# Indra-jith/failure-aware-vision

Hardware: AMD Instinct MI355X
Metric: frames/sec, ResNet-50 MC-Dropout T=30 224x224 batch=256 (higher is better)
Workload: dtype bf16; 1 GPU; BASELINE configs[2]: ResNet-50 v1.5 + MC-Dropout T=30 (all_blocks, p=0.10), 224x224x3 fp32 frames with Gaussian noise severity 3, batch 256 per GPU, synthetic frames and seeded synthetic weights; frames_per_gpu=256, global_batch=256, mc_samples=30, dropout_policy=all_blocks, inputs=resident in HBM before the timed region (H2D excluded), parallelism=batch sharded, 1 process per GPU, all-gather of (label, confidence)

## Files before the change

failure_aware_vision_amd/_lib.py:

```python
from __future__ import annotations

import ctypes as C
import os

_HERE = os.path.dirname(os.path.abspath(__file__))
LIB_PATH = os.environ.get("FAV_LIB_PATH") or os.path.join(_HERE, "lib", "libfav_hip.so")

FAV_OK = 0
STATUS_NAMES = {0: "FAV_OK", 1: "FAV_ERR_INVALID_ARG", 2: "FAV_ERR_BAD_BLOB", 3: "FAV_ERR_NO_WEIGHTS",
                4: "FAV_ERR_HIP", 5: "FAV_ERR_NO_DEVICE", 6: "FAV_ERR_UNSUPPORTED"}
LAYOUT_NHWC_U8, LAYOUT_NHWC_F32 = 0, 1
ARCH_RESNET18_CIFAR, ARCH_RESNET50, ARCH_VIT_B16, ARCH_VIT_TINY = 0, 1, 2, 3
CONF_MAX_SOFTMAX, CONF_ENTROPY, CONF_MUTUAL_INFO = 0, 1, 2
MATH_BF16, MATH_F32_EXACT = 0, 1
K_STEM, K_CONV, K_MAXPOOL, K_AVGPOOL, K_DROPOUT, K_HEAD, K_COUNT = 0, 1, 2, 3, 4, 5, 6
KERNEL_CLASS_NAMES = ("stem_im2col", "conv_igemm", "maxpool", "avgpool", "entry_dropout", "head")


class FavConfig(C.Structure):
    _fields_ = [
        ("struct_size", C.c_uint32), ("device", C.c_int32), ("arch", C.c_int32), ("num_classes", C.c_int32),
        ("in_h", C.c_int32), ("in_w", C.c_int32), ("max_batch", C.c_int32),
        ("mean", C.c_float * 3), ("stdev", C.c_float * 3),
        ("n_samples", C.c_int32), ("site_mask", C.c_uint32), ("dropout_p", C.c_float), ("seed", C.c_uint64),
# ... 13 lines not shown
                ("n_frames", C.c_int32), ("H", C.c_int32), ("W", C.c_int32), ("Cin", C.c_int32), ("Cout", C.c_int32),
                ("kh", C.c_int32), ("kw", C.c_int32), ("stride", C.c_int32), ("pad", C.c_int32),
                ("relu", C.c_int32), ("out_f32", C.c_int32), ("math_mode", C.c_int32), ("drop", FavDropoutDesc)]


class FavLinearDesc(C.Structure):
    _fields_ = [("x", C.c_void_p), ("w", C.c_void_p), ("bias", C.c_void_p), ("res", C.c_void_p), ("y", C.c_void_p),
                ("rows", C.c_int64), ("K", C.c_int32), ("N", C.c_int32), ("act", C.c_int32)]


class FavTailDesc(C.Structure):
    _fields_ = [("x", C.c_void_p), ("wb", C.c_void_p), ("bias_b", C.c_void_p), ("wc", C.c_void_p), ("bias_c", C.c_void_p),
                ("res", C.c_void_p), ("y", C.c_void_p), ("wa", C.c_void_p), ("bias_a", C.c_void_p), ("t1n", C.c_void_p),
                ("n_frames", C.c_int32), ("H", C.c_int32), ("W", C.c_int32), ("Cmid", C.c_int32), ("Nred", C.c_int32),
                ("drop", FavDropoutDesc), ("res_entry", C.c_int32), ("entry_site", C.c_int32)]


class FavUncertainty(C.Structure):
    _fields_ = [("label", C.c_int32), ("confidence", C.c_float), ("mean_prob", C.c_float), ("prob_std", C.c_float),
                ("pred_entropy", C.c_float), ("expected_entropy", C.c_float), ("mutual_info", C.c_float),
                ("agreement", C.c_float), ("top_label", C.c_int32 * 5), ("top_prob", C.c_float * 5)]


CP_LAC, CP_APS = 0, 1


class FavConformal(C.Structure):
    _fields_ = [("struct_size", C.c_uint32), ("score_kind", C.c_int32), ("randomized", C.c_int32), ("k_reg", C.c_int32),
                ("lambda_", C.c_float), ("qhat", C.c_float), ("seed", C.c_uint64)]

# ... 32 lines not shown
                                      C.c_void_p, C.c_void_p]),
    "fav_classify_uncertainty": (C.c_int, [C.c_void_p, C.c_void_p, C.c_int32, C.c_int32, C.c_int64, C.c_void_p, C.c_void_p,
                                          C.c_void_p, C.c_void_p]),
    "fav_classify_sets": (C.c_int, [C.c_void_p, C.c_void_p, C.c_int32, C.c_int32, C.c_int64, C.POINTER(FavConformal),
                                    C.c_void_p, C.c_void_p, C.c_void_p, C.c_void_p]),
    "fav_conformal_scores": (C.c_int, [C.c_void_p, C.c_void_p, C.c_int32, C.c_int32, C.c_int64, C.POINTER(FavConformal),
                                       C.c_void_p, C.c_void_p, C.c_void_p]),
    "fav_classify_host": (C.c_int, [C.c_void_p, C.c_void_p, C.c_int32, C.c_int32, C.c_int64, C.c_void_p, C.c_void_p,
                                    C.c_void_p, C.c_void_p]),
    "fav_get_logits": (C.c_int, [C.c_void_p, C.c_void_p, C.POINTER(C.c_int32), C.POINTER(C.c_int32), C.c_void_p]),
    "fav_set_profiling": (C.c_int, [C.c_void_p, C.c_int32]),
    "fav_get_profile": (C.c_int, [C.c_void_p, C.POINTER(FavProfile), C.c_int32]),
    "fav_get_op_profile": (C.c_int, [C.c_void_p, C.POINTER(FavOpProfile), C.c_int32, C.POINTER(C.c_int32)]),
    "fav_op_conv2d": (C.c_int, [C.POINTER(FavConvDesc), C.c_void_p]),
    "fav_op_bottleneck_tail": (C.c_int, [C.POINTER(FavTailDesc), C.c_void_p]),
    "fav_op_linear_streamk": (C.c_int, [C.POINTER(FavLinearDesc), C.c_void_p]),
    "fav_op_stem_im2col": (C.c_int, [C.c_void_p, C.c_int32, C.c_int32, C.c_int32, C.c_int32, C.c_int32, C.c_int32,
                                     C.c_int32, C.c_int32, C.c_int32, C.POINTER(C.c_float), C.POINTER(C.c_float),
                                     C.c_void_p, C.c_void_p]),
    "fav_op_stem_pool": (C.c_int, [C.c_void_p, C.c_int32, C.c_int32, C.c_int32, C.c_int32, C.c_void_p, C.c_void_p, C.c_void_p, C.c_void_p, C.c_void_p, C.c_void_p]),
    "fav_op_maxpool3x3s2": (C.c_int, [C.c_void_p, C.c_void_p, C.c_int32, C.c_int32, C.c_int32, C.c_int32, C.c_void_p]),
    "fav_op_avgpool": (C.c_int, [C.c_void_p, C.c_void_p, C.c_int32, C.c_int32, C.c_int32, C.POINTER(FavDropoutDesc),
                                 C.c_void_p]),
    "fav_op_entry_dropout": (C.c_int, [C.c_void_p, C.c_void_p, C.c_int64, C.c_int32, C.POINTER(FavDropoutDesc),
                                       C.c_void_p]),
    "fav_op_entry_reduce": (C.c_int, [C.c_void_p, C.c_void_p, C.c_void_p, C.c_void_p, C.c_void_p, C.c_int32, C.c_int32, C.c_int32,
                                      C.c_int32, C.POINTER(FavDropoutDesc), C.c_void_p]),
    "fav_op_layernorm": (C.c_int, [C.c_void_p, C.c_int64, C.c_void_p, C.c_void_p, C.c_void_p, C.c_int64, C.c_int32, C.c_float,
                                   C.c_void_p]),
    "fav_op_attention": (C.c_int, [C.c_void_p, C.c_void_p, C.c_int32, C.c_int32, C.c_int32, C.c_int32, C.c_int32, C.c_void_p]),
# ... 42 lines not shown
```

failure_aware_vision_amd/csrc/fav.hip:

```cpp
#include <hip/hip_runtime.h>

#include <algorithm>
#include <atomic>
#include <cmath>
#include <cstdarg>
#include <cstdio>
#include <cstdlib>
#include <cstring>
#include <string>
#include <vector>

#include "../../include/fav.h"
#include "fav_kernels.hpp"

namespace {

thread_local std::string g_create_error;

std::string fmt(const char* f, ...) {
    char buf[512];
    va_list ap;
    va_start(ap, f);
    vsnprintf(buf, sizeof buf, f, ap);
    va_end(ap);
// ... 393 lines not shown
        } else if (epi && pp && MODE_ == 0) hipLaunchKernelGGL((conv_igemm_kernel<256, 256, 64, 2, 0, 2, 0, 1, 1>), grid, dim3(512), 0, s, p); \
        else if (epi) hipLaunchKernelGGL((conv_igemm_kernel<256, 256, 64, 2, MODE_, 2, 0, 1>), grid, dim3(512), 0, s, p);    \
        else hipLaunchKernelGGL((conv_igemm_kernel<256, 256, 64, 2, MODE_, 2, 0, 0>), grid, dim3(512), 0, s, p);        \
    } while (0)
    if (big) {
        if (d.math_mode == FAV_MATH_BF16) FAV_LAUNCH_BIG(0); else FAV_LAUNCH_BIG(1);
    } else if (d.math_mode == FAV_MATH_BF16) FAV_LAUNCH_MODE(0); else FAV_LAUNCH_MODE(1);
#undef FAV_LAUNCH_BIG
#undef FAV_LAUNCH_MODE
#undef FAV_LAUNCH
    dbg_report(tiles, BM, BN, BK);
    return nullptr;
}


struct TailGeom { int patch_bytes, rega_bytes, lds_bytes, nw, wc2, rp, bias_b_off, bias_ca_off, wa_off0, wa_off1, zero_off; };
bool tail_l4() {
    return FAV_KNOB("FAV_TAIL_L4", 1) != 0;
}
bool tail_geometry(int cmid, int nred, bool has3x3, int W, TailGeom* g) {
    const int cout = 4 * cmid;
    auto finish = [&](int bias_b_off, int wa_off0, int wa_bytes) {
        g->bias_b_off = bias_b_off; g->bias_ca_off = bias_b_off + cmid * 5;
        g->wa_off0 = wa_off0; g->wa_off1 = wa_off0 + wa_bytes;
        g->zero_off = (bias_b_off + (cmid + cout + nred) * 5 + 255) & ~255;
        g->lds_bytes = g->zero_off + 256;
    };
    if (cmid == 512) {
        if (has3x3 || nred != 0) return false;
        g->patch_bytes = 0; g->rega_bytes = 0; g->nw = 8; g->rp = 32; g->wc2 = 1;
        finish(2 * 65536, 2 * 65536, 0);
        return true;
    }
    else if (cmid == 256) { if ((has3x3 && nred != 0) || !(nred == 0 || nred == 256)) return false; }
    else if ((cmid != 64 && cmid != 128) || !(nred == 0 || nred == cmid || nred == 128)) return false;
    if (cmid == 256 && has3x3) {
        g->patch_bytes = 0; g->rega_bytes = 128 * 1024; g->nw = 8; g->rp = 32; g->wc2 = 1;
        finish(g->rega_bytes, g->rega_bytes, 0);
        return true;
    }
    const int rp = (cmid == 256 && nred == 256) ? 16 : 32;
    const int rowb = cmid * 2, ns = cmid == 64 ? 3 : 2;
    const int wc_bytes = 64 * rowb, wa_bytes = nred * 128;
    auto plan = [&](int nw) {
        const int bm = rp * nw;
        const int patch = has3x3 ? (int)((((long long)(bm + 2 * W + 2) * rowb) + 1023) / 1024 * 1024) : 0;
        int rega = has3x3 ? std::max(std::max(patch, bm * 128), bm * rowb) : (nred > 0 ? bm * 128 : 0);
        rega = (rega + 1023) / 1024 * 1024;
        const int ring = has3x3 ? ns * cmid * 128 : 0;
        const int budget = nw == 4 ? 80 * 1024 : 160 * 1024;
        g->patch_bytes = patch; g->rega_bytes = rega; g->nw = nw; g->rp = rp;
        g->wc2 = 1;
        int regb = std::max(ring, 2 * wc_bytes + 2 * wa_bytes);
        finish(rega + regb, rega + 2 * wc_bytes, wa_bytes);
        if (g->lds_bytes > budget) {
            g->wc2 = 0;
            regb = std::max(ring, wc_bytes + 2 * wa_bytes);
            finish(rega + regb, rega + wc_bytes, wa_bytes);
        }
        return g->lds_bytes <= budget;
    };
    return plan((cmid == 128 || (cmid == 256 && nred == 256)) ? 8 : 4);
}

bool tail_wide() {
    return FAV_KNOB("FAV_TAIL_WIDE", 1) != 0;
}

bool tail_wide3x3() {
    return FAV_KNOB("FAV_TAIL_WIDE3X3", 1) != 0;
}

bool tail_enabled() {
    return FAV_KNOB("FAV_FUSE", 1) != 0;
}

const char* launch_tail(fav_handle* h, const fav_tail_desc& d, hipStream_t s) {
    const bool has3x3 = d.wb != nullptr;
    const int nred = d.wa ? d.Nred : 0;
    TailGeom g;
    if (!tail_geometry(d.Cmid, nred, has3x3, d.W, &g)) return "bottleneck tail: unsupported shape";
    const long long M = (long long)d.n_frames * d.H * d.W;
    if (M <= 0 || M > 0x7fffffffLL) return "bottleneck tail: row count out of range";
    TailParams p;
    p.t1 = (const uint16_t*)d.x; p.wb = (const uint16_t*)d.wb; p.bias_b = d.bias_b;
    p.wc = (const uint16_t*)d.wc; p.bias_c = d.bias_c; p.res = (const uint16_t*)d.res; p.y = (uint16_t*)d.y;
    p.wa = (const uint16_t*)d.wa; p.bias_a = d.bias_a; p.t1n = (uint16_t*)d.t1n;
    p.H = d.H; p.W = d.W; p.HW = d.H * d.W; p.M = (int)M;
    p.in_W = d.W; p.in_HW = p.HW; p.in_stride = 1;
    p.rega_bytes = g.rega_bytes;
    p.bias_b_off = g.bias_b_off; p.bias_ca_off = g.bias_ca_off; p.wa_off0 = g.wa_off0; p.wa_off1 = g.wa_off1; p.zero_off = g.zero_off;
    p.drop = make_drop(&d.drop);
    p.div_hw = fastdiv_make((uint32_t)p.HW);
    p.div_w = fastdiv_make((uint32_t)d.W);
    if (p.drop.site >= 0 && (p.drop.v0 < 0 || p.drop.v0 + d.n_frames > 0x7fffffffLL)) return "bottleneck tail: virtual frame index out of range";
    const fav_handle::Group G = h ? h->grp : fav_handle::Group{};
// ... 60 lines not shown
        dbg_report();                                                                                                 \
        return nullptr;                                                                                               \
    } while (0)
#define FAV_TAIL_W(CMID_, NRED_, H3_, NS_, NW_) do { if (g.wc2) FAV_TAIL(CMID_, NRED_, H3_, NS_, NW_, true); else FAV_TAIL(CMID_, NRED_, H3_, NS_, NW_, false); } while (0)
#define FAV_TAIL_N(CMID_, NRED_, H3_, NS_) FAV_TAIL_W(CMID_, NRED_, H3_, NS_, 4)
    if (d.res_entry) {
        const bool sample_minor = FAV_KNOB("FAV_ENTRY_RES_ORDER", 1) != 0;
        const long long sample_rows = (long long)p.drop.n_img * p.HW;
        if (sample_minor && p.drop.v0 % p.drop.n_img == 0 && d.n_frames % p.drop.n_img == 0 && sample_rows % bm == 0) {
            p.rs_T = d.n_frames / p.drop.n_img;
            p.rs_tps = (int)(sample_rows / bm);
        }
        static DeviceFlags attr_set;
        auto k0 = bottleneck_tail_kernel<64, 64, true, 3, 4, false, 32, 0, true, true, true>;
        auto k1 = bottleneck_tail_kernel<64, 64, true, 3, 4, true, 32, 0, true, true, true>;
        if (!attr_set.test_current()) {
            if (hipFuncSetAttribute((const void*)k0, hipFuncAttributeMaxDynamicSharedMemorySize, 160 * 1024) != hipSuccess ||
                hipFuncSetAttribute((const void*)k1, hipFuncAttributeMaxDynamicSharedMemorySize, 160 * 1024) != hipSuccess)
                return "bottleneck tail: cannot reserve LDS";
            attr_set.set_current();
        }
        if (g.wc2) hipLaunchKernelGGL(k1, grid, dim3(256), g.lds_bytes, s, p, g.patch_bytes);
        else hipLaunchKernelGGL(k0, grid, dim3(256), g.lds_bytes, s, p, g.patch_bytes);
        dbg_report();
        return nullptr;
    }
    if (cmid == 64) {
        if (has3x3) { if (nred == 0) FAV_TAIL_N(64, 0, true, 3); if (nred == 64) FAV_TAIL_N(64, 64, true, 3); if (nred == 128) FAV_TAIL_N(64, 128, true, 3); }
        else { if (nred == 0) FAV_TAIL_N(64, 0, false, 3); if (nred == 64) FAV_TAIL_N(64, 64, false, 3); if (nred == 128) FAV_TAIL_N(64, 128, false, 3); }
    } else if (cmid == 128) {
        if (has3x3) { if (nred == 0) FAV_TAIL_W(128, 0, true, 2, 8); if (nred == 128) FAV_TAIL_W(128, 128, true, 2, 8); }
        else { if (nred == 0) FAV_TAIL_W(128, 0, false, 2, 8); if (nred == 128) FAV_TAIL_W(128, 128, false, 2, 8); }
    } else if (cmid == 512) {
        FAV_TAIL(512, 0, false, 2, 8, true);
    } else if (nred == 0 && has3x3) {
        FAV_TAIL(256, 0, true, 2, 8, true);
    } else if (nred == 0) {
        FAV_TAIL_W(256, 0, false, 2, 4);
// ... 1494 lines not shown
    return FAV_OK;
}

fav_status fav_op_conv2d(const fav_conv_desc* d, void* stream) {
    if (!d || !d->x || !d->w || !d->bias || !d->y) return op_done("fav_op_conv2d: null pointer");
    if (d->Cout % 64 != 0) return op_done("fav_op_conv2d: Cout must be a multiple of 64");
    return op_done(launch_conv(nullptr, *d, d->Cout, d->Cout, (hipStream_t)stream));
}

fav_status fav_op_bottleneck_tail(const fav_tail_desc* d, void* stream) {
    if (!d || !d->x || !d->wc || !d->bias_c || !d->res || !d->y) return op_done("fav_op_bottleneck_tail: null pointer");
    if ((d->wb && !d->bias_b) || (d->wa && (!d->bias_a || !d->t1n))) return op_done("fav_op_bottleneck_tail: null pointer");
    return op_done(launch_tail(nullptr, *d, (hipStream_t)stream));
}

fav_status fav_op_stem_im2col(const void* images, int32_t layout, int32_t n, int32_t H, int32_t W, int32_t kh, int32_t kw,
                              int32_t stride, int32_t pad, int32_t kpad, const float* mean3, const float* inv_std3,
                              void* out, void* stream) {
    if (!images || !out || !mean3 || !inv_std3 || kpad % 64 != 0 || kpad < kh * kw * 3) return op_done("fav_op_stem_im2col: bad argument");
    launch_stem(nullptr, images, layout, n, H, W, kh, kw, stride, pad, kpad, mean3, inv_std3, out, (hipStream_t)stream);
    return op_done(nullptr);
}

fav_status fav_op_stem_pool(const void* images, int32_t layout, int32_t n, int32_t H, int32_t W, const void* w, const float* bias,
                            const float* mean3, const float* inv_std3, void* out, void* stream) {
    if (!images || !w || !bias || !mean3 || !inv_std3 || !out) return op_done("fav_op_stem_pool: null argument");
    return op_done(launch_stem_pool(nullptr, images, layout, n, H, W, w, bias, mean3, inv_std3, out, (hipStream_t)stream));
}

fav_status fav_op_maxpool3x3s2(const void* x, void* y, int32_t n, int32_t H, int32_t W, int32_t C, void* stream) {
// ... 101 lines not shown
```

failure_aware_vision_amd/csrc/fav_kernels.hpp:

```cpp
#pragma once
#include <hip/hip_runtime.h>
#include <stdint.h>

#ifdef FAV_EXPERIMENTS
#define FAV_DBG(P) ((P).dbg)
#else
#define FAV_DBG(P) ((unsigned long long*)nullptr)
#endif

namespace fav {

typedef __attribute__((__vector_size__(8 * sizeof(__bf16)))) __bf16 bf16x8_t;
typedef __attribute__((__vector_size__(4 * sizeof(float)))) float f32x4_t;

__device__ __forceinline__ float bf16_bits_to_f32(uint32_t b) { return __uint_as_float(b << 16); }

__device__ __forceinline__ uint32_t f32_to_bf16_bits(float f) {
    uint32_t u = __float_as_uint(f);
    return (u + 0x7FFFu + ((u >> 16) & 1u)) >> 16;
}
typedef __bf16 bf16x2_t __attribute__((ext_vector_type(2)));
typedef float f32x2_t __attribute__((ext_vector_type(2)));
typedef uint32_t u32x4_t __attribute__((ext_vector_type(4)));
__device__ __forceinline__ uint32_t pack_bf16x2(float lo, float hi) {
// ... 1215 lines not shown
        asm volatile("s_waitcnt lgkmcnt(0)" ::: "memory");      \
        __builtin_amdgcn_s_barrier();                           \
        asm volatile("" ::: "memory");                          \
    } while (0)

__device__ __forceinline__ int tail_row_perm(int r) {
    const int g = r & ~63, a = (r >> 4) & 3, i = r & 15;
    return g + 16 * (i >> 2) + 4 * a + (i & 3);
}

template <int CPR>
__device__ __forceinline__ int tail_sw(int row) {
    return CPR == 8 ? (row & 7) : (CPR == 16 ? ((row & 7) | ((row & 1) << 3)) : (row & 15));
}

template <int CMID, int NRED, bool HAS3X3, int NS, int NW, bool WC2, int RP = 32, int COUT_ = 0, bool HAS_RES = true, bool RELU = true, bool RESE = false>
__global__ __launch_bounds__(NW * 64, 2) void bottleneck_tail_kernel(const TailParams p_launch, int patch_bytes) {
    const TailParams p = tail_group_params(p_launch);
    constexpr bool LINEST = NRED > 0 || (HAS3X3 && !(HAS3X3 && CMID == 256));
    constexpr int COUT = COUT_ > 0 ? COUT_ : 4 * CMID;
    static_assert(HAS_RES || (!HAS3X3 && NRED == 0), "only conv_c alone runs without a residual");
    constexpr int BM = RP * NW, NT = NW * 64;
    static_assert(RP == 32 || (RP == 16 && !HAS3X3), "rows per wave");
    constexpr int ROWB = CMID * 2;
    constexpr int CPR = ROWB / 16;
    constexpr int PROWS = 1024 / ROWB;
    constexpr int CB = CMID / 64;
    constexpr int NKT = 9 * CB;
    constexpr int TM = 4;
    constexpr int WN1 = 2;
    constexpr int TN1 = CMID / WN1 / 16;
    constexpr int SLOT = CMID * 128;
    constexpr int BR = SLOT / 1024 / NW;
    constexpr int NCHUNK = COUT / 64;
    constexpr int KS2 = CMID / 32;
    constexpr int TM2 = RP / 16;
    constexpr int G3 = NRED / 64;
    constexpr int WC_BYTES = 64 * ROWB;
    constexpr int WA_BYTES = NRED * 128;
    constexpr int WCN = (HAS3X3 && CMID == 256) ? 4 : (WC2 ? 2 : 1);
    constexpr int BARQ = WCN == 4 ? 2 : 1;
    constexpr int P2W = WCN * WC_BYTES + 2 * WA_BYTES;
    constexpr int RING = HAS3X3 ? NS * SLOT : 0;
    constexpr int REGB = RING > P2W ? RING : P2W;
    constexpr int WC_PIECES = WC_BYTES / 1024, WA_PIECES = WA_BYTES / 1024;
    constexpr int WC_PW = (WC_PIECES + NW - 1) / NW, WA_PW = (WA_PIECES + NW - 1) / NW;
    static_assert(BR >= 1 && TN1 >= 1 && TM2 >= 1 && WC_PIECES % NW == 0 && (NRED == 0 || WA_PIECES % NW == 0), "tile shape");
    static_assert(!HAS3X3 || (NKT % NS == 0 && WC_BYTES <= SLOT), "Wc buffer 0 = ring slot 0, free during the last NS - 1 steps");
    const bool WA0_EARLY = !HAS3X3 || p.wa_off1 >= p.rega_bytes + RING;
    constexpr bool P1G = HAS3X3 && CMID == 256;
    static_assert(!P1G || (NW == 8 && NS == 2 && RP == 32 && NRED == 0 && WC2), "generic conv_b: 8 waves, two stages, conv_c alone behind it");
    extern __shared__ __attribute__((aligned(16))) unsigned char tsm[];
    unsigned char* const ych = tsm;
    unsigned char* const regb = P1G ? tsm : tsm + p.rega_bytes;
    float* const bias_b_s = (float*)(tsm + p.bias_b_off);
    float* const bias_c_s = (float*)(tsm + p.bias_ca_off);
    float* const bias_a_s = bias_c_s + (COUT / 16) * 20;
    const uint32_t zero_off = (uint32_t)p.zero_off;

    const int tid = threadIdx.x, lane = tid & 63, wave = tid >> 6;
    const int wm = wave / WN1, wn = wave % WN1;
    const int wave_u = __builtin_amdgcn_readfirstlane(wave);
    const int frow = lane & 15, fq = lane >> 4;
// ... 39 lines not shown
        }                                                                                                         \
    } while (0)
    if (tid < 64) ((uint32_t*)(tsm + zero_off))[tid] = 0u;
    const __amdgpu_buffer_rsrc_t srd_res = RESE
        ? __builtin_amdgcn_make_buffer_rsrc((void*)p.res, 0, (int)((long long)p.drop.n_img * p.HW * COUT * 2), 0x00020000)
        : __builtin_amdgcn_make_buffer_rsrc((void*)((HAS_RES ? p.res : p.y) + (long long)m0 * COUT), 0, rows_valid * COUT * 2, 0x00020000);
    uint32_t eoff[TM2];
    if constexpr (RESE) {
#pragma unroll
        for (int b = 0; b < TM2; ++b) {
            const uint32_t m = (uint32_t)(m0 + wave * RP + b * 16 + frow);
            const uint32_t vl = fastdiv(m, p.div_hw);
            const uint32_t v = (uint32_t)p.drop.v0 + vl;
            const uint32_t il = v - fastdiv(v, p.drop.div_img) * (uint32_t)p.drop.n_img;
            eoff[b] = m < (uint32_t)p.M ? (il * (uint32_t)p.HW + (m - vl * (uint32_t)p.HW)) * (uint32_t)(COUT * 2) : 0x80000000u;
        }
    }
    u32x4_t rnext[TM2][2];
#define FAV_T_LOAD_RES(J)                                                                                        \
    if (HAS_RES) _Pragma("unroll") for (int b = 0; b < TM2; ++b) {                                               \
        const int off = RESE ? (int)(eoff[b] + (uint32_t)(((J) * 64 + fq * 16) * 2))                             \
                             : ((wave * RP + b * 16 + frow) * COUT + (J) * 64 + fq * 16) * 2;                    \
        rnext[b][0] = __builtin_amdgcn_raw_buffer_load_b128(srd_res, off, 0, 0);                                 \
        rnext[b][1] = __builtin_amdgcn_raw_buffer_load_b128(srd_res, off + 16, 0, 0);                            \
    }
    FAV_T_LOAD_RES(0)
    const uint32_t lds_base =
        __builtin_amdgcn_readfirstlane((uint32_t)(uintptr_t)(const __attribute__((address_space(3))) void*)tsm);
    const uint32_t lds_regb = lds_base + (P1G ? 0u : (uint32_t)p.rega_bytes);
    constexpr uint32_t OOB = 0x80000000u;
    const int wrow = lane >> 3, wch = (lane & 7) ^ (wrow & 7);
    const __amdgpu_buffer_rsrc_t srd_wc = __builtin_amdgcn_make_buffer_rsrc((void*)p.wc, 0, COUT * CMID * 2, 0x00020000);
    const __amdgpu_buffer_rsrc_t srd_wa = __builtin_amdgcn_make_buffer_rsrc((void*)p.wa, 0, NRED > 0 ? NRED * COUT * 2 : 16, 0x00020000);
#define FAV_T_STAGE_WC(J)                                                                                        \
    do {                                                                                                         \
        _Pragma("unroll") for (int i = 0; i < WC_PW; ++i) {                                                      \
            const int pc = wave_u + i * NW;                 \
            const int sub = pc >> 3, r0 = (pc & 7) * 8;                                                          \
            lds_dma16(srd_wc, (uint32_t)((((J) * 64 + tail_row_perm(r0 + wrow)) * CMID + sub * 64 + wch * 8) * 2), 0u, \
                      __builtin_amdgcn_readfirstlane(lds_regb + (uint32_t)(((J) % WCN) * WC_BYTES + pc * 1024)));  \
        }                                                                                                        \
    } while (0)
#define FAV_T_STAGE_WA(J)                                                                                        \
    do {                                                                                                         \
        _Pragma("unroll") for (int i = 0; i < WA_PW; ++i) {                                                      \
            const int pc = wave_u + i * NW;                                                                      \
            lds_dma16(srd_wa, (uint32_t)((tail_row_perm(pc * 8 + wrow) * COUT + wch * 8) * 2), (uint32_t)((J) * 128), \
                      __builtin_amdgcn_readfirstlane(lds_base + (uint32_t)(((((J) + 1) & 1) ? p.wa_off1 : p.wa_off0) + pc * 1024))); \
        }                                                                                                        \
    } while (0)

    const int W = p.W;
    if (NRED > 0 && WA0_EARLY) FAV_T_STAGE_WA(0);
    if (HAS3X3) {
        f32x4_t acc[TN1][TM];
// ... 161 lines not shown
#pragma unroll
                    for (int b = 0; b < TM; ++b) {
                        union { uint4 u; bf16x8_t v; } ua, ub;
                        ua.u = fw[a];
                        ub.u = fx[b];
                        acc[a][b] = __builtin_amdgcn_mfma_f32_16x16x32_bf16(ua.v, ub.v, acc[a][b], 0, 0, 0);
                    }
            }
            if (++cb == CB) {
                cb = 0;
                ++tap;
                if (++ts == 3) { ts = 0; ++tr; }
                tapoff = tr * W + ts;
            }
            if (kt + NS - 1 < NKT) asm volatile("s_waitcnt vmcnt(%0)" ::"n"((NS - 2) * BR) : "memory");
            else if (kt + 1 < NKT) asm volatile("s_waitcnt vmcnt(%0)" ::"n"(WC_PW + (NS - 3) * BR) : "memory");
            __syncthreads();
            cur = (cur + 1 == NS) ? 0 : cur + 1;
            nxt = (nxt + 1 == NS) ? 0 : nxt + 1;
        }
#undef FAV_T_HSTAGE
        }
        if (NRED > 0 && !WA0_EARLY) FAV_T_STAGE_WA(0);
        if (FAV_DBG(p) && tid == 0) FAV_DBG(p)[blockIdx.x * 16ull + 2] = wall_clock64();
#pragma unroll
        for (int a = 0; a < TN1; ++a)
#pragma unroll
            for (int b = 0; b < TM; ++b) {
                const int row = wm * 64 + b * 16 + frow;
                const int c0 = wn * (CMID / WN1) + a * 16 + fq * 4;
                const float4 bq = *(const float4*)(bias_b_s + (c0 >> 4) * 20 + (c0 & 15));
// ... 55 lines not shown
    for (int b = 0; b < TM2; ++b) {
        const uint32_t m = (uint32_t)(m0 + wave * RP + b * 16 + frow);
        const uint32_t vl = fastdiv(m, p.div_hw);
        drop_v[b] = (uint32_t)p.drop.v0 + vl;
        drop_pix[b] = m - vl * (uint32_t)p.HW;
    }
    constexpr int NA3 = NRED > 0 ? NRED / 16 : 1;
    f32x4_t acc3[NA3][TM2];
#pragma unroll
    for (int a = 0; a < NA3; ++a)
#pragma unroll
        for (int b = 0; b < TM2; ++b) acc3[a][b] = (f32x4_t){0.f, 0.f, 0.f, 0.f};

#pragma unroll
    for (int j = 0; j < NCHUNK; ++j) {
        const unsigned char* const wcb = regb + (j % WCN) * WC_BYTES;
        const unsigned char* const wab = tsm + (((j + 1) & 1) ? p.wa_off1 : p.wa_off0);
        if ((j == 1 || j == 2) && FAV_DBG(p) && tid == 0) FAV_DBG(p)[blockIdx.x * 16ull + (j == 1 ? 12 : 14)] = __builtin_amdgcn_s_memtime();
        if (HAS_RES) {
#pragma unroll
            for (int b = 0; b < TM2; ++b) {
                asm volatile("" : "+v"(rnext[b][0]), "+v"(rnext[b][1]));
                rcur[b][0] = rnext[b][0];
                rcur[b][1] = rnext[b][1];
            }
        }
        if (j == 1 && FAV_DBG(p) && tid == 0) { asm volatile("s_nop 0" :: "v"(rcur[TM2 - 1][1])); FAV_DBG(p)[blockIdx.x * 16ull + 13] = __builtin_amdgcn_s_memtime(); }
        if (j + 1 < NCHUNK) {
            if (BARQ == 2) {
                if ((j & 1) == 0 && j + 2 < NCHUNK) { FAV_T_STAGE_WC(j + 2); FAV_T_STAGE_WC(j + 3); }
            } else if (WC2) FAV_T_STAGE_WC(j + 1);
            if (NRED > 0) FAV_T_STAGE_WA(j + 1);
            FAV_T_LOAD_RES(j + 1)
        }
        if (j == 1 && FAV_DBG(p) && tid == 0) FAV_DBG(p)[blockIdx.x * 16ull + 6] = __builtin_amdgcn_s_memtime();
        f32x4_t acc2[4][TM2];
#pragma unroll
        for (int a = 0; a < 4; ++a)
#pragma unroll
            for (int b = 0; b < TM2; ++b) acc2[a][b] = (f32x4_t){0.f, 0.f, 0.f, 0.f};
#pragma unroll
        for (int ks = 0; ks < KS2; ++ks) {
            uint4 fw[4];
#pragma unroll
            for (int a = 0; a < 4; ++a) {
                const int row = a * 16 + frow;
                fw[a] = *(const uint4*)(wcb + (ks >> 1) * 8192 + row * 128 + ((((ks & 1) * 4 + fq) ^ (row & 7)) << 4));
            }
#pragma unroll
            for (int a = 0; a < 4; ++a)
#pragma unroll
                for (int b = 0; b < TM2; ++b) {
                    union { uint4 u; bf16x8_t v; } ua, ub;
                    ua.u = fw[a];
                    ub.u = t2f[b][ks];
                    acc2[a][b] = __builtin_amdgcn_mfma_f32_16x16x32_bf16(ua.v, ub.v, acc2[a][b], 0, 0, 0);
                }
        }
        if (j == 1 && FAV_DBG(p) && tid == 0) { asm volatile("s_nop 0" :: "v"(acc2[3][TM2 - 1])); FAV_DBG(p)[blockIdx.x * 16ull + 7] = __builtin_amdgcn_s_memtime(); }
        if (!WC2 && j + 1 < NCHUNK) {
            FAV_BAR();
            FAV_T_STAGE_WC(j + 1);
        }
        {
            float bia[16];
#pragma unroll
            for (int q = 0; q < 4; ++q) {
                const float4 bq = *(const float4*)(bias_c_s + (j * 4 + fq) * 20 + 4 * q);
                bia[4 * q] = bq.x; bia[4 * q + 1] = bq.y; bia[4 * q + 2] = bq.z; bia[4 * q + 3] = bq.w;
            }
#pragma unroll
            for (int b = 0; b < TM2; ++b) {
                const int row = wave * RP + b * 16 + frow;
                const int n = j * 64 + fq * 16;
                uint32_t draws[4] = {~0u, ~0u, ~0u, ~0u};
                uint32_t edraws[4] = {~0u, ~0u, ~0u, ~0u};
                if (p.drop.site >= 0) {
                    const uint32_t chunk = (uint32_t)(((long long)drop_pix[b] * COUT + n) >> 4);
                    const uint4 w4 = drop_draws16(p.drop, drop_v[b], chunk);
                    draws[0] = w4.x; draws[1] = w4.y; draws[2] = w4.z; draws[3] = w4.w;
                    if constexpr (RESE) {
                        DropParams de = p.drop;
                        de.site = p.site_e;
                        const uint4 e4 = drop_draws16(de, drop_v[b], chunk);
                        edraws[0] = e4.x; edraws[1] = e4.y; edraws[2] = e4.z; edraws[3] = e4.w;
                    }
                }
#pragma unroll
                for (int g = 0; g < 2; ++g) {
                    float v[8];
#pragma unroll
                    for (int k = 0; k < 8; ++k) v[k] = __fadd_rn(acc2[2 * g + (k >> 2)][b][k & 3], bia[8 * g + k]);
                    if (HAS_RES) {
                        uint32_t rw[4] = {rcur[b][g][0], rcur[b][g][1], rcur[b][g][2], rcur[b][g][3]};
                        if constexpr (RESE) {
#pragma unroll
                            for (int k = 0; k < 4; ++k) {
                                const float lo = FAV_DROP_APPLY(bf16_bits_to_f32(rw[k] & 0xFFFFu), edraws, 8 * g + 2 * k, p.drop);
                                const float hi = FAV_DROP_APPLY(bf16_bits_to_f32(rw[k] >> 16), edraws, 8 * g + 2 * k + 1, p.drop);
                                rw[k] = pack_bf16x2(lo, hi);
                            }
                        }
#pragma unroll
                        for (int k = 0; k < 4; ++k) {
                            v[2 * k] = __fadd_rn(v[2 * k], bf16_bits_to_f32(rw[k] & 0xFFFFu));
                            v[2 * k + 1] = __fadd_rn(v[2 * k + 1], bf16_bits_to_f32(rw[k] >> 16));
                        }
                    }
                    if (p.drop.site >= 0) {
#pragma unroll
                        for (int k = 0; k < 8; ++k) v[k] = FAV_DROP_APPLY(v[k], draws, 8 * g + k, p.drop);
                    }
                    u32x4_t o = {pack_bf16x2(v[0], v[1]), pack_bf16x2(v[2], v[3]), pack_bf16x2(v[4], v[5]), pack_bf16x2(v[6], v[7])};
                    if (RELU) {
#pragma unroll
                        for (int k = 0; k < 4; ++k) o[k] = relu_bf16x2(o[k]);
                    }
                    if (!LINEST) __builtin_amdgcn_raw_buffer_store_b128(o, srd_y, (row * COUT + n + 8 * g) * 2, 0, 0);
                    if (LINEST) *(u32x4_t*)(ych + row * 128 + (((2 * fq + g) ^ (row & 7)) << 4)) = o;
                }
            }
        }
        if (j == 1 && FAV_DBG(p) && tid == 0) FAV_DBG(p)[blockIdx.x * 16ull + 8] = __builtin_amdgcn_s_memtime();
        if constexpr (LINEST) {
            asm volatile("s_waitcnt lgkmcnt(0)" ::: "memory");
            {
#pragma unroll
                for (int i = 0; i < TM2 * 2; ++i) {
                    const int row = wave * RP + i * 8 + (lane >> 3);
                    const u32x4_t o = *(const u32x4_t*)(ych + row * 128 + (((lane & 7) ^ (row & 7)) << 4));
                    __builtin_amdgcn_raw_buffer_store_b128(o, srd_y, (row * COUT + j * 64 + (lane & 7) * 8) * 2, 0, 0);
                }
            }
        }
        if constexpr (NRED > 0) {
// ... 9 lines not shown
                for (int a = 0; a < NA3; ++a) {
                    const int row = a * 16 + frow;
                    union { uint4 u; bf16x8_t v; } ua;
                    ua.u = *(const uint4*)(wab + row * 128 + (((ks * 4 + fq) ^ (row & 7)) << 4));
#pragma unroll
                    for (int b = 0; b < TM2; ++b) {
                        union { uint4 u; bf16x8_t v; } ub;
                        ub.u = fy[b];
                        acc3[a][b] = __builtin_amdgcn_mfma_f32_16x16x32_bf16(ua.v, ub.v, acc3[a][b], 0, 0, 0);
                    }
                }
            }
        }
        if (j == 1 && FAV_DBG(p) && tid == 0) { asm volatile("s_nop 0" :: "v"(acc3[NA3 - 1][TM2 - 1])); FAV_DBG(p)[blockIdx.x * 16ull + 9] = __builtin_amdgcn_s_memtime(); }
        if (j + 1 < NCHUNK && (BARQ == 1 || (j & 1))) {
            asm volatile("s_waitcnt vmcnt(%0)" ::"n"((WC2 && HAS_RES) ? 4 * TM2 : 2 * TM2) : "memory");
            if (j == 1 && FAV_DBG(p) && tid == 0) FAV_DBG(p)[blockIdx.x * 16ull + 10] = __builtin_amdgcn_s_memtime();
            FAV_BAR();
            if (j == 1 && FAV_DBG(p) && tid == 0) FAV_DBG(p)[blockIdx.x * 16ull + 11] = __builtin_amdgcn_s_memtime();
        }
    }
#undef FAV_T_LOAD_RES
#undef FAV_T_STAGE_WC
#undef FAV_T_STAGE_WA
#undef FAV_T_BIAS_TO_LDS

    if (FAV_DBG(p) && tid == 0) FAV_DBG(p)[blockIdx.x * 16ull + 4] = wall_clock64();
    if constexpr (NRED > 0) {
        const __amdgpu_buffer_rsrc_t srd_t =
            __builtin_amdgcn_make_buffer_rsrc((void*)(p.t1n + (long long)m0 * NRED), 0, rows_valid * NRED * 2, 0x00020000);
#pragma unroll
        for (int g3 = 0; g3 < G3; ++g3) {
            float bia[16];
#pragma unroll
            for (int q = 0; q < 4; ++q) {
                const float4 bq = *(const float4*)(bias_a_s + (g3 * 4 + fq) * 20 + 4 * q);
                bia[4 * q] = bq.x; bia[4 * q + 1] = bq.y; bia[4 * q + 2] = bq.z; bia[4 * q + 3] = bq.w;
// ... 1494 lines not shown
```

include/fav.h:

```cpp
#ifndef FAV_H
#define FAV_H

#include <stddef.h>
#include <stdint.h>

#ifdef __cplusplus
extern "C" {
#endif

#define FAV_ABI_VERSION 2

typedef struct fav_handle fav_handle;

typedef enum fav_status {
    FAV_OK = 0,
    FAV_ERR_INVALID_ARG = 1,
    FAV_ERR_BAD_BLOB = 2,
    FAV_ERR_NO_WEIGHTS = 3,
    FAV_ERR_HIP = 4,
    FAV_ERR_NO_DEVICE = 5,
    FAV_ERR_UNSUPPORTED = 6
} fav_status;

typedef enum fav_layout { FAV_LAYOUT_NHWC_U8 = 0, FAV_LAYOUT_NHWC_F32 = 1 } fav_layout;
// ... 129 lines not shown
fav_status fav_op_conv2d(const fav_conv_desc* d, void* hip_stream);

typedef struct fav_tail_desc {
    const void* x;
    const void* wb; const float* bias_b;
    const void* wc; const float* bias_c;
    const void* res;
    void* y;
    const void* wa; const float* bias_a;
    void* t1n;
    int32_t n_frames, H, W, Cmid, Nred;
    fav_dropout_desc drop;
    int32_t res_entry, entry_site;
} fav_tail_desc;
fav_status fav_op_bottleneck_tail(const fav_tail_desc* d, void* hip_stream);
fav_status fav_op_stem_im2col(const void* images, int32_t layout, int32_t n, int32_t H, int32_t W,
                              int32_t kh, int32_t kw, int32_t stride, int32_t pad, int32_t kpad,
                              const float* mean3, const float* inv_std3, void* out, void* hip_stream);
fav_status fav_op_stem_pool(const void* images, int32_t layout, int32_t n, int32_t H, int32_t W, const void* w, const float* bias,
                            const float* mean3, const float* inv_std3, void* out, void* hip_stream);
fav_status fav_op_maxpool3x3s2(const void* x, void* y, int32_t n, int32_t H, int32_t W, int32_t C, void* hip_stream);
fav_status fav_op_avgpool(const void* x, void* y, int32_t n, int32_t HW, int32_t C,
                          const fav_dropout_desc* drop, void* hip_stream);
fav_status fav_op_entry_dropout(const void* x, void* out, int64_t elems_per_frame, int32_t n_out,
                                const fav_dropout_desc* drop, void* hip_stream);
fav_status fav_op_entry_reduce(const void* x, void* y, const void* wa, const float* bias_a, void* t1, int32_t C, int32_t Nred,
                               int32_t HW, int32_t n_out, const fav_dropout_desc* drop, void* hip_stream);
fav_status fav_op_head(const float* logits, int32_t T, int32_t n, int32_t num_classes, int32_t ld,
                       float temperature, int32_t conf_kind, float tau,
                       int32_t* labels, float* conf, uint8_t* fail, float* score, void* hip_stream);
// ... 44 lines not shown
```

Baseline: 3427 frames/s.

## Add three-blocks-per-CU LDS plan for cmid=64 bottleneck tail kernel

Adds a tighter LDS geometry for the cmid=64, nred=64 bottleneck tail with a 3x3 conv. It uses two ring slots, a single Wc buffer placed in a ring slot, and launch bounds of occupancy 3, so three blocks fit per CU within 160KB of LDS. To keep register pressure down, residual loads move later, per row block, after the conv_c MMA, and Wa staging is deferred with schedule barriers. This is the default path for layer1 shapes, and a knob and API let callers force 2 or 3 blocks. The trade-off is less load latency hiding from the shallower pipeline and a possible register-limit spill under the 3-block bound.

```diff
diff --git a/failure_aware_vision_amd/_lib.py b/failure_aware_vision_amd/_lib.py
--- a/failure_aware_vision_amd/_lib.py
+++ b/failure_aware_vision_amd/_lib.py
@@ -51,6 +51,11 @@
                 ("res", C.c_void_p), ("y", C.c_void_p), ("wa", C.c_void_p), ("bias_a", C.c_void_p), ("t1n", C.c_void_p),
                 ("n_frames", C.c_int32), ("H", C.c_int32), ("W", C.c_int32), ("Cmid", C.c_int32), ("Nred", C.c_int32),
                 ("drop", FavDropoutDesc), ("res_entry", C.c_int32), ("entry_site", C.c_int32)]
+
+
+class FavTailPlan(C.Structure):
+    _fields_ = [(k, C.c_int32) for k in ("lds_bytes", "patch_bytes", "rega_bytes", "waves", "rows_per_wave", "ring_slots", "wc_buffers",
+                                         "blocks_per_cu", "bias_b_off", "bias_ca_off", "wa_off0", "wa_off1", "zero_off")]
 
 
 class FavUncertainty(C.Structure):
@@ -113,6 +118,8 @@
     "fav_get_op_profile": (C.c_int, [C.c_void_p, C.POINTER(FavOpProfile), C.c_int32, C.POINTER(C.c_int32)]),
     "fav_op_conv2d": (C.c_int, [C.POINTER(FavConvDesc), C.c_void_p]),
     "fav_op_bottleneck_tail": (C.c_int, [C.POINTER(FavTailDesc), C.c_void_p]),
+    "fav_op_bottleneck_tail_plan": (C.c_int, [C.POINTER(FavTailDesc), C.c_int32, C.c_void_p]),
+    "fav_tail_lds_plan": (C.c_int, [C.c_int32, C.c_int32, C.c_int32, C.c_int32, C.c_int32, C.POINTER(FavTailPlan)]),
     "fav_op_linear_streamk": (C.c_int, [C.POINTER(FavLinearDesc), C.c_void_p]),
     "fav_op_stem_im2col": (C.c_int, [C.c_void_p, C.c_int32, C.c_int32, C.c_int32, C.c_int32, C.c_int32, C.c_int32,
                                      C.c_int32, C.c_int32, C.c_int32, C.POINTER(C.c_float), C.POINTER(C.c_float),
diff --git a/failure_aware_vision_amd/csrc/fav.hip b/failure_aware_vision_amd/csrc/fav.hip
--- a/failure_aware_vision_amd/csrc/fav.hip
+++ b/failure_aware_vision_amd/csrc/fav.hip
@@ -431,12 +431,29 @@
 }
 
 
-struct TailGeom { int patch_bytes, rega_bytes, lds_bytes, nw, wc2, rp, bias_b_off, bias_ca_off, wa_off0, wa_off1, zero_off; };
+struct TailGeom { int patch_bytes, rega_bytes, lds_bytes, nw, wc2, rp, bias_b_off, bias_ca_off, wa_off0, wa_off1, zero_off, ns, occ; };
 bool tail_l4() {
     return FAV_KNOB("FAV_TAIL_L4", 1) != 0;
 }
-bool tail_geometry(int cmid, int nred, bool has3x3, int W, TailGeom* g) {
+bool tail_geometry(int cmid, int nred, bool has3x3, int W, TailGeom* g, int blocks = 0) {
     const int cout = 4 * cmid;
+    g->ns = cmid == 64 ? 3 : 2; g->occ = 2;
+    if (blocks != 2 && cmid == 64 && nred == 64 && has3x3) {
+        const int bm = 128, rowb = 128, slot = 8192, wc_bytes = 8192, wa_bytes = 8192, ych = bm * 128;
+        const int patch = (int)((((long long)(bm + 2 * W + 2) * rowb) + 1023) / 1024 * 1024);
+        const int rega = std::max(patch, ych + wa_bytes);
+        const int regb = std::max(2 * slot, slot + wc_bytes);
+        const int bias_b_off = rega + regb;
+        const int zero_off = (bias_b_off + (cmid + cout + nred) * 5 + 255) & ~255;
+        if ((long long)(zero_off + 256) * 3 <= 160 * 1024) {
+            g->patch_bytes = patch; g->rega_bytes = rega; g->nw = 4; g->rp = 32; g->wc2 = 0; g->ns = 2; g->occ = 3;
+            g->bias_b_off = bias_b_off; g->bias_ca_off = bias_b_off + cmid * 5;
+            g->wa_off0 = ych; g->wa_off1 = rega;
+            g->zero_off = zero_off; g->lds_bytes = zero_off + 256;
+            return true;
+        }
+    }
+    if (blocks == 3) return false;
     auto finish = [&](int bias_b_off, int wa_off0, int wa_bytes) {
         g->bias_b_off = bias_b_off; g->bias_ca_off = bias_b_off + cmid * 5;
         g->wa_off0 = wa_off0; g->wa_off1 = wa_off0 + wa_bytes;
@@ -445,14 +462,14 @@
     };
     if (cmid == 512) {
         if (has3x3 || nred != 0) return false;
-        g->patch_bytes = 0; g->rega_bytes = 0; g->nw = 8; g->rp = 32; g->wc2 = 1;
+        g->patch_bytes = 0; g->rega_bytes = 0; g->nw = 8; g->rp = 32; g->wc2 = 1; g->occ = 1;
         finish(2 * 65536, 2 * 65536, 0);
         return true;
     }
     else if (cmid == 256) { if ((has3x3 && nred != 0) || !(nred == 0 || nred == 256)) return false; }
     else if ((cmid != 64 && cmid != 128) || !(nred == 0 || nred == cmid || nred == 128)) return false;
     if (cmid == 256 && has3x3) {
-        g->patch_bytes = 0; g->rega_bytes = 128 * 1024; g->nw = 8; g->rp = 32; g->wc2 = 1;
+        g->patch_bytes = 0; g->rega_bytes = 128 * 1024; g->nw = 8; g->rp = 32; g->wc2 = 1; g->occ = 1;
         finish(g->rega_bytes, g->rega_bytes, 0);
         return true;
     }
@@ -466,7 +483,7 @@
         rega = (rega + 1023) / 1024 * 1024;
         const int ring = has3x3 ? ns * cmid * 128 : 0;
         const int budget = nw == 4 ? 80 * 1024 : 160 * 1024;
-        g->patch_bytes = patch; g->rega_bytes = rega; g->nw = nw; g->rp = rp;
+        g->patch_bytes = patch; g->rega_bytes = rega; g->nw = nw; g->rp = rp; g->occ = nw == 4 ? 2 : 1;
         g->wc2 = 1;
         int regb = std::max(ring, 2 * wc_bytes + 2 * wa_bytes);
         finish(rega + regb, rega + 2 * wc_bytes, wa_bytes);
@@ -492,11 +509,12 @@
     return FAV_KNOB("FAV_FUSE", 1) != 0;
 }
 
-const char* launch_tail(fav_handle* h, const fav_tail_desc& d, hipStream_t s) {
+const char* launch_tail(fav_handle* h, const fav_tail_desc& d, hipStream_t s, int blocks = 0) {
     const bool has3x3 = d.wb != nullptr;
     const int nred = d.wa ? d.Nred : 0;
     TailGeom g;
-    if (!tail_geometry(d.Cmid, nred, has3x3, d.W, &g)) return "bottleneck tail: unsupported shape";
+    if (blocks == 0) blocks = (int)FAV_KNOB("FAV_TAIL_BLOCKS", 0);
+    if (!tail_geometry(d.Cmid, nred, has3x3, d.W, &g, blocks)) return blocks == 3 ? "bottleneck tail: no three-blocks-per-CU plan for this shape" : "bottleneck tail: unsupported shape";
     const long long M = (long long)d.n_frames * d.H * d.W;
     if (M <= 0 || M > 0x7fffffffLL) return "bottleneck tail: row count out of range";
     TailParams p;
@@ -587,14 +605,28 @@
         static DeviceFlags attr_set;
         auto k0 = bottleneck_tail_kernel<64, 64, true, 3, 4, false, 32, 0, true, true, true>;
         auto k1 = bottleneck_tail_kernel<64, 64, true, 3, 4, true, 32, 0, true, true, true>;
+        auto k3 = bottleneck_tail_kernel<64, 64, true, 2, 4, false, 32, 0, true, true, true, 3>;
         if (!attr_set.test_current()) {
             if (hipFuncSetAttribute((const void*)k0, hipFuncAttributeMaxDynamicSharedMemorySize, 160 * 1024) != hipSuccess ||
-                hipFuncSetAttribute((const void*)k1, hipFuncAttributeMaxDynamicSharedMemorySize, 160 * 1024) != hipSuccess)
+                hipFuncSetAttribute((const void*)k1, hipFuncAttributeMaxDynamicSharedMemorySize, 160 * 1024) != hipSuccess ||
+                hipFuncSetAttribute((const void*)k3, hipFuncAttributeMaxDynamicSharedMemorySize, 160 * 1024) != hipSuccess)
                 return "bottleneck tail: cannot reserve LDS";
             attr_set.set_current();
         }
-        if (g.wc2) hipLaunchKernelGGL(k1, grid, dim3(256), g.lds_bytes, s, p, g.patch_bytes);
+        if (g.occ == 3) hipLaunchKernelGGL(k3, grid, dim3(256), g.lds_bytes, s, p, g.patch_bytes);
+        else if (g.wc2) hipLaunchKernelGGL(k1, grid, dim3(256), g.lds_bytes, s, p, g.patch_bytes);
         else hipLaunchKernelGGL(k0, grid, dim3(256), g.lds_bytes, s, p, g.patch_bytes);
+        dbg_report();
+        return nullptr;
+    }
+    if (g.occ == 3) {
+        static DeviceFlags attr_set;
+        auto k3 = bottleneck_tail_kernel<64, 64, true, 2, 4, false, 32, 0, true, true, false, 3>;
+        if (!attr_set.test_current()) {
+            if (hipFuncSetAttribute((const void*)k3, hipFuncAttributeMaxDynamicSharedMemorySize, 160 * 1024) != hipSuccess) return "bottleneck tail: cannot reserve LDS";
+            attr_set.set_current();
+        }
+        hipLaunchKernelGGL(k3, grid, dim3(256), g.lds_bytes, s, p, g.patch_bytes);
         dbg_report();
         return nullptr;
     }
@@ -2119,6 +2151,23 @@
     return op_done(launch_tail(nullptr, *d, (hipStream_t)stream));
 }
 
+fav_status fav_op_bottleneck_tail_plan(const fav_tail_desc* d, int32_t blocks_per_cu, void* stream) {
+    if (!d || !d->x || !d->wc || !d->bias_c || !d->res || !d->y) return op_done("fav_op_bottleneck_tail_plan: null pointer");
+    if ((d->wb && !d->bias_b) || (d->wa && (!d->bias_a || !d->t1n))) return op_done("fav_op_bottleneck_tail_plan: null pointer");
+    if (blocks_per_cu != 0 && blocks_per_cu != 2 && blocks_per_cu != 3) return op_done("fav_op_bottleneck_tail_plan: blocks_per_cu is 0, 2 or 3");
+    return op_done(launch_tail(nullptr, *d, (hipStream_t)stream, blocks_per_cu));
+}
+
+fav_status fav_tail_lds_plan(int32_t Cmid, int32_t Nred, int32_t has3x3, int32_t W, int32_t blocks_per_cu, fav_tail_plan* out) {
+    if (!out || W < 1 || (blocks_per_cu != 0 && blocks_per_cu != 2 && blocks_per_cu != 3)) return FAV_ERR_INVALID_ARG;
+    TailGeom g;
+    if (!tail_geometry(Cmid, Nred, has3x3 != 0, W, &g, blocks_per_cu)) return FAV_ERR_INVALID_ARG;
+    out->lds_bytes = g.lds_bytes; out->patch_bytes = g.patch_bytes; out->rega_bytes = g.rega_bytes;
+    out->waves = g.nw; out->rows_per_wave = g.rp; out->ring_slots = g.ns; out->wc_buffers = g.wc2 ? 2 : 1; out->blocks_per_cu = g.occ;
+    out->bias_b_off = g.bias_b_off; out->bias_ca_off = g.bias_ca_off; out->wa_off0 = g.wa_off0; out->wa_off1 = g.wa_off1; out->zero_off = g.zero_off;
+    return FAV_OK;
+}
+
 fav_status fav_op_stem_im2col(const void* images, int32_t layout, int32_t n, int32_t H, int32_t W, int32_t kh, int32_t kw,
                               int32_t stride, int32_t pad, int32_t kpad, const float* mean3, const float* inv_std3,
                               void* out, void* stream) {
diff --git a/failure_aware_vision_amd/csrc/fav_kernels.hpp b/failure_aware_vision_amd/csrc/fav_kernels.hpp
--- a/failure_aware_vision_amd/csrc/fav_kernels.hpp
+++ b/failure_aware_vision_amd/csrc/fav_kernels.hpp
@@ -1253,8 +1253,9 @@
     return CPR == 8 ? (row & 7) : (CPR == 16 ? ((row & 7) | ((row & 1) << 3)) : (row & 15));
 }
 
-template <int CMID, int NRED, bool HAS3X3, int NS, int NW, bool WC2, int RP = 32, int COUT_ = 0, bool HAS_RES = true, bool RELU = true, bool RESE = false>
-__global__ __launch_bounds__(NW * 64, 2) void bottleneck_tail_kernel(const TailParams p_launch, int patch_bytes) {
+template <int CMID, int NRED, bool HAS3X3, int NS, int NW, bool WC2, int RP = 32, int COUT_ = 0, bool HAS_RES = true, bool RELU = true, bool RESE = false,
+          int OCC = 2>
+__global__ __launch_bounds__(NW * 64, OCC) void bottleneck_tail_kernel(const TailParams p_launch, int patch_bytes) {
     const TailParams p = tail_group_params(p_launch);
     constexpr bool LINEST = NRED > 0 || (HAS3X3 && !(HAS3X3 && CMID == 256));
     constexpr int COUT = COUT_ > 0 ? COUT_ : 4 * CMID;
@@ -1279,13 +1280,16 @@
     constexpr int WA_BYTES = NRED * 128;
     constexpr int WCN = (HAS3X3 && CMID == 256) ? 4 : (WC2 ? 2 : 1);
     constexpr int BARQ = WCN == 4 ? 2 : 1;
+    constexpr bool RES_LATE = OCC >= 3 && HAS_RES;
+    static_assert(!RES_LATE || BARQ == 1, "late residual: one barrier per chunk");
     constexpr int P2W = WCN * WC_BYTES + 2 * WA_BYTES;
     constexpr int RING = HAS3X3 ? NS * SLOT : 0;
     constexpr int REGB = RING > P2W ? RING : P2W;
     constexpr int WC_PIECES = WC_BYTES / 1024, WA_PIECES = WA_BYTES / 1024;
     constexpr int WC_PW = (WC_PIECES + NW - 1) / NW, WA_PW = (WA_PIECES + NW - 1) / NW;
     static_assert(BR >= 1 && TN1 >= 1 && TM2 >= 1 && WC_PIECES % NW == 0 && (NRED == 0 || WA_PIECES % NW == 0), "tile shape");
-    static_assert(!HAS3X3 || (NKT % NS == 0 && WC_BYTES <= SLOT), "Wc buffer 0 = ring slot 0, free during the last NS - 1 steps");
+    constexpr int WC_BASE = HAS3X3 ? (NKT % NS) * SLOT : 0;
+    static_assert(!HAS3X3 || (WC_BYTES <= SLOT && (NKT % NS == 0 || (NKT % NS == NS - 1 && WCN == 1))), "Wc buffer 0 = a ring slot that is free during the last step");
     const bool WA0_EARLY = !HAS3X3 || p.wa_off1 >= p.rega_bytes + RING;
     constexpr bool P1G = HAS3X3 && CMID == 256;
     static_assert(!P1G || (NW == 8 && NS == 2 && RP == 32 && NRED == 0 && WC2), "generic conv_b: 8 waves, two stages, conv_c alone behind it");
@@ -1355,16 +1359,19 @@
             const uint32_t v = (uint32_t)p.drop.v0 + vl;
             const uint32_t il = v - fastdiv(v, p.drop.div_img) * (uint32_t)p.drop.n_img;
             eoff[b] = m < (uint32_t)p.M ? (il * (uint32_t)p.HW + (m - vl * (uint32_t)p.HW)) * (uint32_t)(COUT * 2) : 0x80000000u;
+            if (RES_LATE) eoff[b] += (uint32_t)(fq * 32);
         }
     }
     u32x4_t rnext[TM2][2];
-#define FAV_T_LOAD_RES(J)                                                                                        \
-    if (HAS_RES) _Pragma("unroll") for (int b = 0; b < TM2; ++b) {                                               \
-        const int off = RESE ? (int)(eoff[b] + (uint32_t)(((J) * 64 + fq * 16) * 2))                             \
-                             : ((wave * RP + b * 16 + frow) * COUT + (J) * 64 + fq * 16) * 2;                    \
+#define FAV_T_LOAD_RES_B(J, b)                                                                                   \
+    do {                                                                                                         \
+        const int off = RESE ? (int)(eoff[b] + (uint32_t)(((J) * 64 + (RES_LATE ? 0 : fq * 16)) * 2))            \
+                             : ((wave * RP + (b) * 16 + frow) * COUT + (J) * 64 + fq * 16) * 2;                  \
         rnext[b][0] = __builtin_amdgcn_raw_buffer_load_b128(srd_res, off, 0, 0);                                 \
         rnext[b][1] = __builtin_amdgcn_raw_buffer_load_b128(srd_res, off + 16, 0, 0);                            \
-    }
+    } while (0)
+#define FAV_T_LOAD_RES(J)                                                                                        \
+    if (HAS_RES) _Pragma("unroll") for (int b = 0; b < TM2; ++b) FAV_T_LOAD_RES_B(J, b);
     FAV_T_LOAD_RES(0)
     const uint32_t lds_base =
         __builtin_amdgcn_readfirstlane((uint32_t)(uintptr_t)(const __attribute__((address_space(3))) void*)tsm);
@@ -1379,7 +1386,7 @@
             const int pc = wave_u + i * NW;                 \
             const int sub = pc >> 3, r0 = (pc & 7) * 8;                                                          \
             lds_dma16(srd_wc, (uint32_t)((((J) * 64 + tail_row_perm(r0 + wrow)) * CMID + sub * 64 + wch * 8) * 2), 0u, \
-                      __builtin_amdgcn_readfirstlane(lds_regb + (uint32_t)(((J) % WCN) * WC_BYTES + pc * 1024)));  \
+                      __builtin_amdgcn_readfirstlane(lds_regb + (uint32_t)(WC_BASE + ((J) % WCN) * WC_BYTES + pc * 1024)));  \
         }                                                                                                        \
     } while (0)
 #define FAV_T_STAGE_WA(J)                                                                                        \
@@ -1571,7 +1578,7 @@
                 tapoff = tr * W + ts;
             }
             if (kt + NS - 1 < NKT) asm volatile("s_waitcnt vmcnt(%0)" ::"n"((NS - 2) * BR) : "memory");
-            else if (kt + 1 < NKT) asm volatile("s_waitcnt vmcnt(%0)" ::"n"(WC_PW + (NS - 3) * BR) : "memory");
+            else if (NS > 2 && kt + 1 < NKT) asm volatile("s_waitcnt vmcnt(%0)" ::"n"(WC_PW + (NS - 3) * BR) : "memory");
             __syncthreads();
             cur = (cur + 1 == NS) ? 0 : cur + 1;
             nxt = (nxt + 1 == NS) ? 0 : nxt + 1;
@@ -1657,10 +1664,10 @@
 
 #pragma unroll
     for (int j = 0; j < NCHUNK; ++j) {
-        const unsigned char* const wcb = regb + (j % WCN) * WC_BYTES;
+        const unsigned char* const wcb = regb + WC_BASE + (j % WCN) * WC_BYTES;
         const unsigned char* const wab = tsm + (((j + 1) & 1) ? p.wa_off1 : p.wa_off0);
         if ((j == 1 || j == 2) && FAV_DBG(p) && tid == 0) FAV_DBG(p)[blockIdx.x * 16ull + (j == 1 ? 12 : 14)] = __builtin_amdgcn_s_memtime();
-        if (HAS_RES) {
+        if (HAS_RES && !RES_LATE) {
 #pragma unroll
             for (int b = 0; b < TM2; ++b) {
                 asm volatile("" : "+v"(rnext[b][0]), "+v"(rnext[b][1]));
@@ -1668,13 +1675,13 @@
                 rcur[b][1] = rnext[b][1];
             }
         }
-        if (j == 1 && FAV_DBG(p) && tid == 0) { asm volatile("s_nop 0" :: "v"(rcur[TM2 - 1][1])); FAV_DBG(p)[blockIdx.x * 16ull + 13] = __builtin_amdgcn_s_memtime(); }
+        if (j == 1 && FAV_DBG(p) && tid == 0) { asm volatile("s_nop 0" :: "v"(RES_LATE ? rnext[TM2 - 1][1] : rcur[TM2 - 1][1])); FAV_DBG(p)[blockIdx.x * 16ull + 13] = __builtin_amdgcn_s_memtime(); }
         if (j + 1 < NCHUNK) {
             if (BARQ == 2) {
                 if ((j & 1) == 0 && j + 2 < NCHUNK) { FAV_T_STAGE_WC(j + 2); FAV_T_STAGE_WC(j + 3); }
             } else if (WC2) FAV_T_STAGE_WC(j + 1);
-            if (NRED > 0) FAV_T_STAGE_WA(j + 1);
-            FAV_T_LOAD_RES(j + 1)
+            if (NRED > 0 && !RES_LATE) FAV_T_STAGE_WA(j + 1);
+            if (!RES_LATE) FAV_T_LOAD_RES(j + 1)
         }
         if (j == 1 && FAV_DBG(p) && tid == 0) FAV_DBG(p)[blockIdx.x * 16ull + 6] = __builtin_amdgcn_s_memtime();
         f32x4_t acc2[4][TM2];
@@ -1701,10 +1708,16 @@
                 }
         }
         if (j == 1 && FAV_DBG(p) && tid == 0) { asm volatile("s_nop 0" :: "v"(acc2[3][TM2 - 1])); FAV_DBG(p)[blockIdx.x * 16ull + 7] = __builtin_amdgcn_s_memtime(); }
+        if (RES_LATE) {
+#pragma unroll
+            for (int b = 0; b < TM2; ++b) asm volatile("" : "+v"(rnext[b][0]), "+v"(rnext[b][1]));
+            if (NRED > 0 && j + 1 < NCHUNK) FAV_T_STAGE_WA(j + 1);
+        }
         if (!WC2 && j + 1 < NCHUNK) {
             FAV_BAR();
             FAV_T_STAGE_WC(j + 1);
         }
+        if (OCC >= 3) __builtin_amdgcn_sched_barrier(0);
         {
             float bia[16];
 #pragma unroll
@@ -1718,11 +1731,29 @@
                 const int n = j * 64 + fq * 16;
                 uint32_t draws[4] = {~0u, ~0u, ~0u, ~0u};
                 uint32_t edraws[4] = {~0u, ~0u, ~0u, ~0u};
+                if constexpr (RESE && RES_LATE) {
+                    if (p.drop.site >= 0) {
+                        DropParams de = p.drop;
+                        de.site = p.site_e;
+                        const uint4 e4 = drop_draws16(de, drop_v[b], (uint32_t)(((long long)drop_pix[b] * COUT + n) >> 4));
+                        edraws[0] = e4.x; edraws[1] = e4.y; edraws[2] = e4.z; edraws[3] = e4.w;
+                    }
+#pragma unroll
+                    for (int g = 0; g < 2; ++g)
+#pragma unroll
+                        for (int k = 0; k < 4; ++k) {
+                            const uint32_t r = rnext[b][g][k];
+                            const float lo = FAV_DROP_APPLY(bf16_bits_to_f32(r & 0xFFFFu), edraws, 8 * g + 2 * k, p.drop);
+                            const float hi = FAV_DROP_APPLY(bf16_bits_to_f32(r >> 16), edraws, 8 * g + 2 * k + 1, p.drop);
+                            rnext[b][g][k] = pack_bf16x2(lo, hi);
+                        }
+                    __builtin_amdgcn_sched_barrier(0);
+                }
                 if (p.drop.site >= 0) {
                     const uint32_t chunk = (uint32_t)(((long long)drop_pix[b] * COUT + n) >> 4);
                     const uint4 w4 = drop_draws16(p.drop, drop_v[b], chunk);
                     draws[0] = w4.x; draws[1] = w4.y; draws[2] = w4.z; draws[3] = w4.w;
-                    if constexpr (RESE) {
+                    if constexpr (RESE && !RES_LATE) {
                         DropParams de = p.drop;
                         de.site = p.site_e;
                         const uint4 e4 = drop_draws16(de, drop_v[b], chunk);
@@ -1735,8 +1766,9 @@
 #pragma unroll
                     for (int k = 0; k < 8; ++k) v[k] = __fadd_rn(acc2[2 * g + (k >> 2)][b][k & 3], bia[8 * g + k]);
                     if (HAS_RES) {
-                        uint32_t rw[4] = {rcur[b][g][0], rcur[b][g][1], rcur[b][g][2], rcur[b][g][3]};
-                        if constexpr (RESE) {
+                        const u32x4_t rq = RES_LATE ? rnext[b][g] : rcur[b][g];
+                        uint32_t rw[4] = {rq[0], rq[1], rq[2], rq[3]};
+                        if constexpr (RESE && !RES_LATE) {
 #pragma unroll
                             for (int k = 0; k < 4; ++k) {
                                 const float lo = FAV_DROP_APPLY(bf16_bits_to_f32(rw[k] & 0xFFFFu), edraws, 8 * g + 2 * k, p.drop);
@@ -1762,6 +1794,7 @@
                     if (!LINEST) __builtin_amdgcn_raw_buffer_store_b128(o, srd_y, (row * COUT + n + 8 * g) * 2, 0, 0);
                     if (LINEST) *(u32x4_t*)(ych + row * 128 + (((2 * fq + g) ^ (row & 7)) << 4)) = o;
                 }
+                if (RES_LATE && j + 1 < NCHUNK) FAV_T_LOAD_RES_B(j + 1, b);
             }
         }
         if (j == 1 && FAV_DBG(p) && tid == 0) FAV_DBG(p)[blockIdx.x * 16ull + 8] = __builtin_amdgcn_s_memtime();
@@ -1801,13 +1834,14 @@
         }
         if (j == 1 && FAV_DBG(p) && tid == 0) { asm volatile("s_nop 0" :: "v"(acc3[NA3 - 1][TM2 - 1])); FAV_DBG(p)[blockIdx.x * 16ull + 9] = __builtin_amdgcn_s_memtime(); }
         if (j + 1 < NCHUNK && (BARQ == 1 || (j & 1))) {
-            asm volatile("s_waitcnt vmcnt(%0)" ::"n"((WC2 && HAS_RES) ? 4 * TM2 : 2 * TM2) : "memory");
+            asm volatile("s_waitcnt vmcnt(%0)" ::"n"(((WC2 || RES_LATE) && HAS_RES) ? 4 * TM2 : 2 * TM2) : "memory");
             if (j == 1 && FAV_DBG(p) && tid == 0) FAV_DBG(p)[blockIdx.x * 16ull + 10] = __builtin_amdgcn_s_memtime();
             FAV_BAR();
             if (j == 1 && FAV_DBG(p) && tid == 0) FAV_DBG(p)[blockIdx.x * 16ull + 11] = __builtin_amdgcn_s_memtime();
         }
     }
 #undef FAV_T_LOAD_RES
+#undef FAV_T_LOAD_RES_B
 #undef FAV_T_STAGE_WC
 #undef FAV_T_STAGE_WA
 #undef FAV_T_BIAS_TO_LDS
diff --git a/include/fav.h b/include/fav.h
--- a/include/fav.h
+++ b/include/fav.h
@@ -167,6 +167,12 @@
     int32_t res_entry, entry_site;
 } fav_tail_desc;
 fav_status fav_op_bottleneck_tail(const fav_tail_desc* d, void* hip_stream);
+fav_status fav_op_bottleneck_tail_plan(const fav_tail_desc* d, int32_t blocks_per_cu, void* hip_stream);
+typedef struct fav_tail_plan {
+    int32_t lds_bytes, patch_bytes, rega_bytes, waves, rows_per_wave, ring_slots, wc_buffers, blocks_per_cu;
+    int32_t bias_b_off, bias_ca_off, wa_off0, wa_off1, zero_off;
+} fav_tail_plan;
+fav_status fav_tail_lds_plan(int32_t Cmid, int32_t Nred, int32_t has3x3, int32_t W, int32_t blocks_per_cu, fav_tail_plan* out);
 fav_status fav_op_stem_im2col(const void* images, int32_t layout, int32_t n, int32_t H, int32_t W,
                               int32_t kh, int32_t kw, int32_t stride, int32_t pad, int32_t kpad,
                               const float* mean3, const float* inv_std3, void* out, void* hip_stream);
```

Result: no change. 3448 frames/s (median of 6 runs) (+0.6%).
